# SYNCC-IN/hyperscanning-signal-analysis

Hardware: AMD Instinct MI355X
Metric: MVAR+ffDTF windows/sec, 2x32-ch dyad p=8, 256 freqs (higher is better)
Workload: dtype f64; 1 GPU; C2: 1 dyad(s)/GPU, 2x32 ch @500 Hz, 10 min, 2 s windows 50% overlap (599 windows per dyad), MVAR p=8, 256 freqs 0.5-128 Hz; dyads_per_gpu=1, k1=hop blocks summed once, shared by the overlapping windows (hop 500), k2=block Levinson-Whittle recursion, one workgroup per window, one launch, normalisation=inside K3 (rows of window w by workgroups of window w+lag), parallelism=dyad-sharded x1, gather=none

## Files before the change

hyperscanning_signal_analysis_amd/csrc/capi.hip:

```cpp
#include "../../include/hypermvar.h"
#include "hmv_kernels.h"

#include <atomic>
#include <cmath>
#include <cstdio>
#include <cstdlib>
#include <cstring>

namespace {
thread_local char g_err[256] = "";

int fail(int code, const char* msg) {
  snprintf(g_err, sizeof(g_err), "%s", msg);
  return code;
}
int pad_of(int m) { return (m < 1 || m > HMV_MAX_CHANNELS) ? -1 : ((m + 15) / 16) * 16; }
inline hipStream_t S(void* s) { return reinterpret_cast<hipStream_t>(s); }
inline size_t align256(size_t b) { return (b + 255) & ~size_t(255); }

constexpr int N_TUNE = 6;
struct TuneRange { long long lo, hi; };
constexpr TuneRange kTuneRange[N_TUNE] = {{0, 0}, {0, 1 << 20}, {0, 3}, {0, 2}, {0, 3}, {0, 140000}};
long long env_knob(const char* name, int key) {
  const char* e = getenv(name);
// ... 126 lines not shown
    const int64_t need = ens_q_tiles(n_items, n, p, grid_hop, grid_nwin) * (int64_t)(p + 1) * mp * mp;
    if (!workspace || workspace_doubles < need) return fail(-7, "hmv_lagcov_ensemble_f64: workspace too small");
  }
  hmv::LagcovEnsArgs a{};
  a.x = x; a.rec_stride = rec_stride; a.ld = ld; a.T = T;
  a.trial_rec = reinterpret_cast<const long long*>(trial_rec);
  a.trial_start = reinterpret_cast<const long long*>(trial_start);
  a.group_ptr = reinterpret_cast<const long long*>(group_ptr);
  a.item_group = reinterpret_cast<const long long*>(item_group);
  a.item_offset = reinterpret_cast<const long long*>(item_offset);
  a.n_items = n_items; a.m = m; a.n = n; a.p = p; a.R = R;
  if (shared) { a.it0 = 0; a.nwin = grid_nwin; a.hop = grid_hop; a.k = (int)(n / grid_hop); a.Q = workspace; }
  return hmv::launch_lagcov_ensemble(a, mp, shared, S(stream));
}

int hmv_yw_solve_f64(const double* R, int64_t n_items, int m, int p, double* ws, double* ar, double* V,
                     double* vq_logdet, int32_t* info, int64_t flags, void* stream) {
  const int mp = pad_of(m);
  if (mp < 0) return fail(-1, "hmv_yw_solve_f64: channel count must be in 1..64");
  if (p < 1 || p > HMV_MAX_ORDER) return fail(-2, "hmv_yw_solve_f64: model order must be in 1..32");
  if (!R || !ws || !ar || !V || !info || n_items < 0) return fail(-4, "hmv_yw_solve_f64: null pointer");
  hmv::YwArgs a{};
  a.R = R; a.n_items = n_items; a.m = m; a.p = p; a.ws = ws; a.ar = ar; a.V = V;
  a.Vq_logdet = vq_logdet; a.info = info; a.tiled = (flags & HMV_FLAG_YW_TILED) ? 1 : ((flags & HMV_FLAG_YW_ONE_LAUNCH) ? 0 : -1);
  return hmv::launch_yw(a, mp, S(stream));
}

namespace {
double crit_factor(int crit, int n) {
  return crit == 0 ? 2.0 : (crit == 1 ? 2.0 * log(log((double)n)) : log((double)n));
}
}

int hmv_yw_solve_auto_f64(const double* R, int64_t n_items, int m, int pmax, int n, int crit, double* ws, double* ar,
                          double* V, int32_t* order_out, double* crit_out, double* vq_logdet, int32_t* info, int64_t flags,
                          void* stream) {
  const int mp = pad_of(m);
  if (mp < 0) return fail(-1, "hmv_yw_solve_auto_f64: channel count must be in 1..64");
  if (pmax < 1 || pmax > HMV_MAX_ORDER) return fail(-2, "hmv_yw_solve_auto_f64: largest model order must be in 1..32");
  if (n <= pmax) return fail(-3, "hmv_yw_solve_auto_f64: window shorter than the largest model order");
// ... 197 lines not shown
  if (const int64_t t = hmv::tuning(HMV_TUNE_NORM_LAG)) lag = t;
  return lag < 8 ? 8 : lag;
}
}

int64_t hmv_tf_ffdtf_workspace_bytes(int64_t n_items, int m, int p, int F) {
  const int mp = pad_of(m);
  if (mp < 0 || n_items < 0 || p < 1 || F < 1) return -1;
  return (int64_t)tf_ff_layout(n_items, mp, p, F).total;
}

namespace {
int tf_ffdtf_impl(const char* who, const double* ar, int64_t n_items, int m, int p, const double* tw, int F, double* ffdtf,
                  double* band_out, const int32_t* bin_lo, const int32_t* bin_hi, int n_bands, double* den, double* H,
                  int32_t* info, double pivot_tau, void* workspace, int64_t workspace_bytes, int64_t flags,
                  void* ev_k3_start, void* ev_k3_stop, void* stream) {
  auto failw = [&](int code, const char* msg) {
    char buf[200];
    snprintf(buf, sizeof(buf), "%s: %s", who, msg);
    return fail(code, buf);
  };
  const int mp = pad_of(m);
  const bool bands = (band_out != nullptr);
  if (mp < 0) return failw(-1, "channel count must be in 1..64");
  if (p < 1) return failw(-2, "model order must be >= 1");
  if (n_items == 0) return 0;
  if (!ar || !tw || (!ffdtf && !bands) || !den || !info || !workspace || n_items < 0 || F < 1)
    return failw(-4, "null pointer / empty grid");
  if (!(pivot_tau > 0.0) || pivot_tau > 1.0) return failw(-6, "pivot_tau must be in (0, 1]");
  if (bands) {
    if (!bin_lo || !bin_hi || n_bands < 1) return failw(-4, "band bins missing");
    if (F % 32 != 0 || F > hmv::tf_band_max_F(mp) || (flags & HMV_FLAG_UNFUSED_NORM))
      return failw(-10, "in-kernel band sums need F % 32 == 0, F within the row worker's LDS block and the fused normalisation");
  }
  const TfFfWs w = tf_ff_layout(n_items, mp, p, F, bands);
  if ((int64_t)w.total > workspace_bytes) return failw(-7, "workspace too small");
  char* base = static_cast<char*>(workspace);
  const size_t t = (size_t)mp * mp;
  hmv::TfArgs a{};
  a.ar = ar; a.arx = reinterpret_cast<double*>(base + w.off_arx); a.tw = tw;
  a.P = reinterpret_cast<double*>(base + w.off_P); a.rowsum = reinterpret_cast<double*>(base + w.off_rowsum);
  a.H = H;
  a.info = info; a.n_items = n_items; a.F = F; a.p = p; a.m = m; a.tau = pivot_tau;
  const bool fused = bands || (!(flags & HMV_FLAG_UNFUSED_NORM) && (F % 16 == 0) && (reinterpret_cast<uintptr_t>(ffdtf) % 16 == 0));
  const int64_t lag = norm_lag_items(mp, F);
  const int64_t n_fused = fused ? n_items : 0;
  if (n_fused > 0) {
    a.ff = bands ? nullptr : ffdtf; a.den = den; a.fuse_items = n_fused; a.lag = (int)lag;
    if (bands) {
      a.bands = band_out; a.band_lo = reinterpret_cast<const int*>(bin_lo); a.band_hi = reinterpret_cast<const int*>(bin_hi);
      a.nb = n_bands;
    }
    a.wcount = reinterpret_cast<int*>(base + w.off_cnt);
    a.ready = a.wcount + n_items;
    a.missed = a.ready + n_items;
// ... 195 lines not shown
  double* Qb = reinterpret_cast<double*>(base + w.off_Q);
  double* ws = reinterpret_cast<double*>(base + w.off_ws);
  double* ar = reinterpret_cast<double*>(base + w.off_ar);
  double* V = reinterpret_cast<double*>(base + w.off_V);
  void* tfws = base + w.off_tf;
  double* den = reinterpret_cast<double*>(base + w.off_den);
  double* tw = reinterpret_cast<double*>(base + w.off_tw);
  const bool k3_bands = bands && a.measure == MEAS_FFDTF;
  const int64_t tfws_bytes = (int64_t)tf_ff_layout(a.chunk, mp, a.p, a.F, k3_bands).total;
  rc = hmv_twiddles_f64(a.freqs, a.F, a.fs, a.p, tw, st0);
  const size_t ws_item = (size_t)hmv_yw_workspace_doubles(a.m, a.p);
  for (int64_t ci = 0; ci < n_chunks && rc == 0; ++ci) {
    const int64_t i0 = ci * a.chunk;
    const int64_t c = (a.n_items - i0 < a.chunk) ? (a.n_items - i0) : a.chunk;
    double* ar_c = a.ar_out ? a.ar_out + (size_t)i0 * t * a.p : ar;
    double* V_c = a.V_out ? a.V_out + (size_t)i0 * t : V;
    if (a.ens) {
      hmv::LagcovEnsArgs ea{};
      ea.x = a.x; ea.rec_stride = a.rec_stride; ea.ld = a.ld; ea.T = a.ens->T;
      ea.trial_rec = reinterpret_cast<const long long*>(a.ens->trial_rec);
      ea.trial_start = reinterpret_cast<const long long*>(a.ens->trial_start);
      ea.group_ptr = reinterpret_cast<const long long*>(a.ens->group_ptr);
      ea.item_group = reinterpret_cast<const long long*>(a.item_rec + i0);
      ea.item_offset = reinterpret_cast<const long long*>(a.item_start + i0);
      ea.n_items = c; ea.m = a.m; ea.n = a.n; ea.p = a.p; ea.R = R;
      if (ens_shared) {
        ea.it0 = i0; ea.nwin = a.grid_nwin; ea.hop = a.grid_hop; ea.k = (int)(a.n / a.grid_hop); ea.Q = Qb;
      }
      rc = hmv::launch_lagcov_ensemble(ea, mp, ens_shared, st0);
    } else if (regular) {
// ... 25 lines not shown
    const int64_t c0 = (split && tiled && c >= 16) ? (c + 1) / 2 : c, c1 = c - c0;
    if (c1 > 0 && !automatic) {
      int hrc = (int)hipEventRecord(fj->fork, st0);
      if (!hrc) hrc = (int)hipStreamWaitEvent(st1, fj->fork, 0);
      if (hrc) { rc = hrc; break; }
      rc = hmv_yw_solve_f64(R + (size_t)c0 * (a.p + 1) * t, c1, a.m, a.p, ws + (size_t)c0 * ws_item,
                            ar_c + (size_t)c0 * t * a.p, V_c + (size_t)c0 * t, nullptr, a.info_yw + i0 + c0, yw_flags, st1);
      hrc = (int)hipEventRecord(fj->join, st1);
      if (!hrc) hrc = (int)hipStreamWaitEvent(st0, fj->join, 0);
      if (hrc) {
        (void)hipStreamSynchronize(st1);
        if (!rc) rc = hrc;
      }
      if (rc) break;
    }
    if (!automatic) rc = hmv_yw_solve_f64(R, c0, a.m, a.p, ws, ar_c, V_c, nullptr, a.info_yw + i0, yw_flags, st0);
    if (rc) break;
    const bool last = (ci == n_chunks - 1);
    double* Hc = a.S_out ? reinterpret_cast<double*>(base + w.off_H) : nullptr;
    double* full_c = (a.measure == MEAS_FFDTF) ? nullptr
                     : bands ? reinterpret_cast<double*>(base + w.off_full) : a.ffdtf + (size_t)i0 * a.m * a.m * a.F;
    if (a.measure == MEAS_GPDC) {
      rc = hmv::launch_gpdc_sliding(ar_c, V_c, tw, full_c, c, a.F, a.m, mp, a.p, st0);
    } else {
      rc = tf_ffdtf_impl(a.who, ar_c, c, a.m, a.p, tw, a.F,
                         k3_bands ? nullptr : (full_c ? full_c : a.ffdtf + (size_t)i0 * a.m * a.m * a.F),
                         k3_bands ? a.band_out + (size_t)i0 * a.m * a.m * a.n_bands : nullptr, a.bin_lo, a.bin_hi,
                         a.n_bands, den, Hc, a.info_tf + (size_t)i0 * a.F, a.pivot_tau, tfws, tfws_bytes, a.flags,
                         last ? a.ev_k3_start : nullptr, last ? a.ev_k3_stop : nullptr, st0);
    }
    if (!rc && a.measure == MEAS_DDTF) {
      hmv::DdtfArgs da{};
      da.ar = ar_c; da.V = V_c; da.info_yw = a.info_yw + i0;
      da.B = reinterpret_cast<double*>(base + w.off_B); da.G = reinterpret_cast<double*>(base + w.off_G);
      da.freqs = a.freqs; da.fs = a.fs; da.ff = full_c; da.out = full_c;
      da.n_items = c; da.F = a.F; da.m = a.m; da.p = a.p;
      rc = hmv::launch_ddtf_sliding(da, mp, st0);
    }
    if (!rc && a.measure != MEAS_FFDTF && bands)
      rc = hmv::launch_band_sums(full_c, reinterpret_cast<const int*>(a.bin_lo), reinterpret_cast<const int*>(a.bin_hi),
                                 a.band_out + (size_t)i0 * a.m * a.m * a.n_bands, c * (long long)a.m * a.m, a.F,
                                 a.n_bands, st0);
    if (!rc && a.S_out) {
      hmv::SpecArgs sa;
// ... 293 lines not shown
```

hyperscanning_signal_analysis_amd/csrc/hmv_kernels.h:

```cpp
#pragma once
#include <hip/hip_runtime.h>
#include <stdint.h>

namespace hmv {

long long tuning(int key);

struct LagcovArgs {
  const double* x;
  long long rec_stride;
  long long ld;
  const long long* item_rec;
  const long long* item_start;
  long long n_items;
  int m, n, p;
  double* R;
  int blocks;
  long long blk_first, blk_T;
};
int launch_lagcov(const LagcovArgs& a, int m_pad, hipStream_t st);
struct LagcombArgs {
  const double* Q;
  const double* x;
  long long ld, first, hop, T;
// ... 22 lines not shown
long long lagcov_ensemble_q_tiles(long long n_items, long long nwin, int k);
int launch_lagcov_ensemble(const LagcovEnsArgs& a, int m_pad, bool shared, hipStream_t st);

struct YwArgs {
  const double* R;
  long long n_items;
  int m, p;
  double* ws;
  double* ar;
  double* V;
  double* Vq_logdet;
  int* info;
  int tiled;
  int only_guarded;
  const int* order;
};
struct YwAutoArgs {
  int n;
  double crit_c;
  int* order_out;
  double* crit_out;
};
long long yw_ws_tiles(int p);
int launch_yw(const YwArgs& a, int m_pad, hipStream_t st);
int launch_yw_lwr(const YwArgs& a, int m_pad, hipStream_t st);
int launch_yw_lwr2(const YwArgs& a, int m_pad, hipStream_t st);
int launch_yw_auto(const YwArgs& a, const YwAutoArgs& s, int m_pad, hipStream_t st);
int launch_yw_guarded(const YwArgs& a, int m_pad, hipStream_t st);

struct TfArgs {
  const double* ar;
  const double* arx;
  const double* tw;
  const double* Zin;
  double* detph;
  double* P;
  double* rowsum;
  double* H;
  double* A;
  int* info;
  long long n_items;
  int F, p, m;
  double tau;
  double* ff;
  double* den;
  int* wcount;
  int* ready;
// ... 122 lines not shown
```

hyperscanning_signal_analysis_amd/csrc/tf_inv.hip:

```cpp
#include "hmv_common.h"
#include "hmv_kernels.h"

namespace hmv {

#ifndef HMV_K3_WGS
#define HMV_K3_WGS 4
#endif

#ifndef HMV_ROW_LOADS_SC1
#define HMV_ROW_LOADS_SC1 0
#endif

#define HMV_LDS_FENCE()                                     \
  do {                                                      \
    __builtin_amdgcn_fence(__ATOMIC_RELEASE, "wavefront");  \
    __builtin_amdgcn_wave_barrier();                        \
    __builtin_amdgcn_fence(__ATOMIC_ACQUIRE, "wavefront");  \
  } while (0)

#ifdef HMV_STAMP
#define HMV_T(idx)                                                                     \
  do {                                                                                 \
    __builtin_amdgcn_sched_barrier(0);                                                 \
    unsigned long long t_;                                                             \
// ... 192 lines not shown
        if (b < nbp && b0 + b < nb) {
          const double t0 = row16_sum_dpp(acc[b][0]), t1 = row16_sum_dpp(acc[b][1]);
          if (c == 0 && j0 < m) ow[b] = t0;
          if (c == 0 && j0 + 1 < m) ow[nb + b] = t1;
        }
      }
    }
  }
}

template <int NT>
__global__ void __launch_bounds__(64 * NT) norm_missed_kernel(TfArgs a) {
  __shared__ double lds[2 * TfLds<NT>::TOTAL];
  static_assert(NormLds<NT>::DOUBLES <= 2 * TfLds<NT>::TOTAL, "normaliser tiles do not fit");
  const int n = a.missed[0];
  const long long tail0 = a.fuse_items > a.lag ? a.fuse_items - a.lag : 0;
  const long long total = n + (a.fuse_items - tail0) * a.m;
  for (long long k = blockIdx.x; k < total; k += gridDim.x) {
    int item, i;
    if (k < n) {
      const int e = a.missed[1 + k];
      item = e / (16 * NT);
      i = e % (16 * NT);
    } else {
      const long long r = k - n;
      item = (int)(tail0 + r / a.m);
      i = (int)(r % a.m);
    }
    if (a.bands) band_row<NT>(a, item, i, lds, 2 * TfLds<NT>::TOTAL, (int)threadIdx.x);
    else normalise_row<NT>(a, item, i, lds, (int)threadIdx.x);
    __syncthreads();
  }
}

template <int NT, bool GEN, bool BANDS = true>
__device__ __forceinline__ void tf_outputs(const TfArgs& a, const int item, const int f, const long long gw, const int w,
                                           const int wv, double (&re)[NT][4], double (&im)[NT][4], double2* smem,
                                           double* rsum, const int* s_orig, int* s_flag, const double* s_det
#ifdef HMV_STAMP
                                           , unsigned long long (&tsum)[8], unsigned long long& tlast
#endif
) {
  constexpr int MP = 16 * NT, NG = NT;
  using L = TfLds<NT>;
  constexpr int NR = L::NRING;
  int& s_info = *s_flag;
  int lo;
  asm volatile("v_mbcnt_lo_u32_b32 %0, -1, 0\n\tv_mbcnt_hi_u32_b32 %0, -1, %0" : "=v"(lo));
  const int rowo = 4 * ((lo >> 2) & 3) + (lo >> 4), jo = lo & 3;
  const int tid = 64 * wv + lo;
  int oc[4];
#pragma unroll
  for (int Jl = 0; Jl < 4; ++Jl) oc[Jl] = s_orig[4 * (Jl * NT + w) + jo];
  if (w == 0 && lo == 0) {
    a.info[gw] = s_info;
    if constexpr (GEN) {
      if (a.detph) {
        a.detph[2 * gw] = s_det[0];
        a.detph[2 * gw + 1] = s_det[1];
      }
    }
  }

  if (a.H) {
    double2* Ho = reinterpret_cast<double2*>(a.H) + (size_t)gw * MP * MP + (size_t)rowo * MP;
#pragma unroll
    for (int Ig = 0; Ig < NG; ++Ig)
#pragma unroll
      for (int Jl = 0; Jl < 4; ++Jl) Ho[(size_t)(16 * Ig) * MP + oc[Jl]] = make_double2(re[Ig][Jl], im[Ig][Jl]);
  }
  if (a.P) {
    double* rs = rsum + w * MP + rowo;
    const bool publish = !GEN && (a.ff != nullptr || a.bands != nullptr) && item < a.fuse_items;
    if (!publish) {
      double* Po = a.P + (size_t)gw * MP * MP + (size_t)rowo * MP;
#pragma unroll
      for (int Ig = 0; Ig < NG; ++Ig) {
        double acc = 0.0;
#pragma unroll
        for (int Jl = 0; Jl < 4; ++Jl) {
          const double v = re[Ig][Jl] * re[Ig][Jl] + im[Ig][Jl] * im[Ig][Jl];
          Po[(size_t)(16 * Ig) * MP + oc[Jl]] = v;
          acc += v;
        }
        acc += dpp_f64<0xB1>(acc);
        acc += dpp_f64<0x4E>(acc);
// ... 59 lines not shown
            __builtin_amdgcn_fence(__ATOMIC_ACQUIRE, "agent");
            asm volatile("s_waitcnt vmcnt(0)" ::: "memory");
          }
          s_info = last;
        }
        __syncthreads();
        HMV_T(5);
        if (s_info != 0) {
          window_denominators<NT>(a, item, nlds, tid);
          asm volatile("s_waitcnt vmcnt(0)" ::: "memory");
          __syncthreads();
          if (tid == 0) __hip_atomic_store(a.ready + item, 1, __ATOMIC_RELAXED, __HIP_MEMORY_SCOPE_AGENT);
        }
      }
      const int wl = item - a.lag;
      if (wl >= 0 && wl < a.fuse_items - a.lag && f < a.m) {
        __syncthreads();
        if (tid == 0) {
          const int rdy = __hip_atomic_load(a.ready + wl, __ATOMIC_RELAXED, __HIP_MEMORY_SCOPE_AGENT);
          if (!rdy) {
            for (int i = f; i < a.m; i += a.F) {
              const int pos = __hip_atomic_fetch_add(a.missed, 1, __ATOMIC_RELAXED, __HIP_MEMORY_SCOPE_AGENT);
              a.missed[1 + pos] = wl * MP + i;
            }
          }
          s_info = rdy;
        }
        __syncthreads();
        HMV_T(6);
        if (s_info != 0) {
          if (BANDS && a.bands) {
            if constexpr (BANDS)
              for (int i = f; i < a.m; i += a.F) band_row<NT>(a, wl, i, nlds, 2 * L::TOTAL, tid);
          } else {
            for (int i = f; i < a.m; i += a.F) normalise_row<NT>(a, wl, i, nlds, tid);
          }
        }
      }
    }
  }
#ifdef HMV_STAMP
  HMV_T(7);
  if (a.stamps && lo == 0) {
    for (int k = 0; k < 8; ++k) a.stamps[(gw * NT + wv) * 8 + k] = tsum[k];
  }
#endif
}

template <int NT, bool GEN>
__global__ void __launch_bounds__(64 * NT, (NT == 4) ? HMV_K3_WGS : 2) tf_inv_kernel(TfArgs a) {
  constexpr int MP = 16 * NT, NG = NT, NSTEP = MP / 4;
  using L = TfLds<NT>;
  constexpr int NR = L::NRING;
  __shared__ double2 smem[L::TOTAL];
  __shared__ int s_orig[MP];
  __shared__ __attribute__((aligned(16))) int s_swp[NR][4];
  __shared__ int s_info;
  __shared__ double s_det[2];

  const int l = lane_id();
  const int wv = uni(threadIdx.x >> 6);
  const int w = (wv + (int)((blockIdx.x * 2654435761u) >> 20)) % NT;
  const int item = uni((int)(blockIdx.x / (unsigned)a.F));
  const int f = uni((int)(blockIdx.x - (unsigned)item * (unsigned)a.F));
  const long long gw = (long long)item * a.F + f;
  const int p = a.p;
  const int i = l >> 4, b = (l >> 2) & 3, j = l & 3;
  const int rowl = 4 * b + i;
  const int colw = 4 * w + j;

  double2* Pbuf = smem;
  double2* Nbuf = Pbuf + L::PBUF;
  double2* Srow = Nbuf + NR * L::NBUF;
  double2* swapb = Srow + L::SROW + wv * 32;
  double* rsum = reinterpret_cast<double*>(Srow + L::SROW + L::SWAPB);

  double re[NG][4], im[NG][4];
#ifdef HMV_STAMP
  unsigned long long tsum[8] = {0, 0, 0, 0, 0, 0, 0, 0}, tlast;
  asm volatile("s_memtime %0\n\ts_waitcnt lgkmcnt(0)" : "=s"(tlast)::"memory");
#endif

  if constexpr (GEN) {
    const double2* Zi = reinterpret_cast<const double2*>(a.Zin) + (size_t)gw * MP * MP + (size_t)rowl * MP + colw;
#pragma unroll
    for (int Ig = 0; Ig < NG; ++Ig)
#pragma unroll
      for (int Jl = 0; Jl < 4; ++Jl) {
        const double2 v = Zi[(size_t)(16 * Ig) * MP + 4 * NT * Jl];
        re[Ig][Jl] = v.x;
        im[Ig][Jl] = v.y;
      }
  } else {
    const int P2 = (p + 1) >> 1;
    const double2* ax = reinterpret_cast<const double2*>(a.arx) +
                        ((size_t)item * NT + w) * (size_t)(NG * 4 * 64) * P2 + l;
    const double* tw = a.tw + (size_t)f * p * 2;
#pragma unroll
    for (int Ig = 0; Ig < NG; ++Ig)
#pragma unroll
      for (int Jl = 0; Jl < 4; ++Jl) {
        re[Ig][Jl] = (16 * Ig + rowl == 4 * NT * Jl + colw) ? 1.0 : 0.0;
        im[Ig][Jl] = 0.0;
      }
    auto chunk = [&](auto hc_tag, int h0) __attribute__((always_inline)) {
      constexpr int HC = decltype(hc_tag)::value;
      constexpr int NB = NG * 4, DEPTH = (HC == 4) ? 3 : 8;
      double zr[2 * HC], zi[2 * HC];
// ... 241 lines not shown
        HMV_LDS_FENCE();
      }
    }
  };
  auto take_panel = [&](auto tc, auto jc) __attribute__((always_inline)) {
    constexpr int t = decltype(tc)::value, J = decltype(jc)::value;
    const double2* Nt = Nbuf + (t % NR) * L::NBUF;
#pragma unroll
    for (int Ig = 0; Ig < NG; ++Ig) {
      const double2 v = Nt[(16 * Ig + rowl) * 4 + j];
      re[Ig][J] = v.x;
      im[Ig][J] = v.y;
    }
  };

  if (w == 0) factor_panel(std::integral_constant<int, 0>{}, std::integral_constant<int, 0>{});
  HMV_T(1);
  __syncthreads();
  HMV_T(2);
  static_for<NSTEP>([&](auto sc) __attribute__((always_inline)) {
    constexpr int s = decltype(sc)::value;
    constexpr int own = s % NT, Js = s / NT;
    constexpr bool has_next = (s + 1 < NSTEP);
    constexpr int nxt = (s + 1) % NT, Jn = has_next ? (s + 1) / NT : 0;
    if (has_next && w == nxt) __builtin_amdgcn_s_setprio(3);
    if constexpr (s >= 1) {
      constexpr int t = s - 1;
      double ar_[NG], ai_[NG];
#pragma unroll
      for (int Ig = 0; Ig < NG; ++Ig) ar_[Ig] = ai_[Ig] = 0.0;
      if (w == own) load_n(std::integral_constant<int, t>{}, ar_, ai_);
      static_for<4>([&](auto jc) __attribute__((always_inline)) {
        constexpr int Jl = decltype(jc)::value;
        if constexpr (Jl != Js && !(NT == 1 && Jl == t / NT)) {
          if (w == own) update_block(std::integral_constant<int, t>{}, jc, ar_, ai_);
        }
      });
    }
    HMV_T(3);
    __builtin_amdgcn_sched_barrier(0);
    double nr[NG], ni[NG];
    load_n(sc, nr, ni);
    interchange(sc);
    HMV_T(3);
    const bool is_nxt = has_next && (w == nxt);
    if (w == own) take_panel(sc, std::integral_constant<int, Js>{});
    if (is_nxt || !(w == own && Jn == Js)) update_block(sc, std::integral_constant<int, Jn>{}, nr, ni);
    static_for<4>([&](auto jc) __attribute__((always_inline)) {
      constexpr int Jl = decltype(jc)::value;
      if constexpr (Jl != Jn) {
        if (!is_nxt && !(w == own && Jl == Js)) update_block(sc, jc, nr, ni);
      }
    });
    HMV_T(3);
    __builtin_amdgcn_sched_barrier(0);
    if (is_nxt) factor_panel(std::integral_constant<int, s + 1>{}, std::integral_constant<int, Jn>{});
    HMV_T(1);
    __syncthreads();
    HMV_T(2);
  });

  HMV_T(3);
  tf_outputs<NT, GEN, (NT < 4)>(a, item, f, gw, w, wv, re, im, smem, rsum, s_orig, &s_info, s_det
#ifdef HMV_STAMP
                      , tsum, tlast
#endif
  );
}

#ifndef HMV_K3A_INC
#define HMV_K3A_INC "tf_inv64_body.inc"
#endif
#include HMV_K3A_INC
#ifndef HMV_K3A_WGS
#ifdef HMV_STAMP
// ... 15 lines not shown
  const int item = uni((int)(blockIdx.x / (unsigned)a.F));
  const int f = uni((int)(blockIdx.x - (unsigned)item * (unsigned)a.F));
  const long long gw = (long long)item * a.F + f;
  if (w == 0) {
    const int l = lane_id();
    s_orig[l] = l;
    if (l == 0) *s_flag = 0;
  }
  const int p = a.p, P2 = (p + 1) >> 1;
  const double* arx = a.arx + ((size_t)item * NT + w) * (size_t)(16 * 64 * 2) * P2;
  const double* tw = a.tw + (size_t)f * p * 2;
  const double tau = a.tau;
  const unsigned ldsbase = (unsigned)(uintptr_t)lds;
  double acc[32];
#ifdef HMV_STAMP
  unsigned long long tsum[8] = {0, 0, 0, 0, 0, 0, 0, 0}, tlast = 0, q0, q1, q2, q3;
  unsigned tl32;
  K3A_BODY_STAMPED(acc, arx, tw, p, w, tau, ldsbase, q0, q1, q2, q3, tl32);
  {
    const unsigned long long d[8] = {q0 & 0xffffffffull, q0 >> 32, q1 & 0xffffffffull, q1 >> 32,
                                     q2 & 0xffffffffull, q2 >> 32, q3 & 0xffffffffull, q3 >> 32};
    tsum[0] = d[0]; tsum[2] = d[1]; tsum[3] = d[2] + d[3] + d[4]; tsum[1] = d[5] + d[6] + d[7];
    unsigned long long now;
    asm volatile("s_memtime %0\n\ts_waitcnt lgkmcnt(0)" : "=s"(now)::"memory");
    tlast = (now & ~0xffffffffull) | tl32;
    if (tlast > now) tlast -= 0x100000000ull;
    if (a.stamps && lane_id() == 0) {
      unsigned long long* det = a.stamps + ((size_t)a.n_items * a.F * NT + (size_t)(gw * NT + wv)) * 8;
      for (int k = 0; k < 8; ++k) det[k] = d[k];
    }
  }
#else
  K3A_BODY(acc, arx, tw, p, w, tau, ldsbase);
#endif
  double re[NT][4], im[NT][4];
#pragma unroll
  for (int Ig = 0; Ig < 4; ++Ig)
#pragma unroll
    for (int Jl = 0; Jl < 4; ++Jl) {
      re[Ig][Jl] = acc[2 * (4 * Ig + Jl)];
      im[Ig][Jl] = acc[2 * (4 * Ig + Jl) + 1];
    }
  double2* smem = reinterpret_cast<double2*>(lds);
  double* rsum = reinterpret_cast<double*>(lds + K3A_RSUM);
  tf_outputs<NT, false>(a, item, f, gw, w, wv, re, im, smem, rsum, s_orig, s_flag, nullptr
#ifdef HMV_STAMP
                        , tsum, tlast
#endif
// ... 48 lines not shown
    case 64: return (2 * TfLds<4>::TOTAL) & ~31;
  }
  return 0;
}

long long tf_workspace_doubles(long long n_items, int m_pad, int p) {
  return n_items * (long long)m_pad * m_pad * 2 * ((p + 1) / 2);
}

int launch_tf_inv(const TfArgs& a_in, int m_pad, hipStream_t st, hipEvent_t ev_start, hipEvent_t ev_stop) {
  TfArgs a = a_in;
  if (a.n_items == 0 || a.F == 0) return 0;
  const bool fused = ((a.ff != nullptr || a.bands != nullptr) && a.fuse_items > 0);
  if (fused) {
    if (!a.P || !a.den || !a.wcount || !a.ready || !a.missed || a.lag < 1) return -3;
    if (a.bands && (!a.band_lo || !a.band_hi || a.nb < 1 || a.F % 32 != 0 || a.F > tf_band_max_F(m_pad) || a.A)) return -3;
    if (const hipError_t e = hipMemsetAsync(a.wcount, 0, sizeof(int) * (2 * (size_t)a.n_items + 1), st)) return (int)e;
  } else {
    a.ff = nullptr;
    a.bands = nullptr;
  }
  const long long n = a.n_items * (long long)a.F;
  const dim3 grid((unsigned)n);
  const long long slots = a.n_items * (long long)m_pad * m_pad * ((a.p + 1) / 2);
  const dim3 pgrid((unsigned)((slots + 255) / 256));
  double* arx = const_cast<double*>(a.arx);
  switch (m_pad) {
    case 16: hipLaunchKernelGGL(ar_pack_kernel<1>, pgrid, dim3(256), 0, st, a.ar, arx, a.n_items, a.p); break;
    case 32: hipLaunchKernelGGL(ar_pack_kernel<2>, pgrid, dim3(256), 0, st, a.ar, arx, a.n_items, a.p); break;
    case 48: hipLaunchKernelGGL(ar_pack_kernel<3>, pgrid, dim3(256), 0, st, a.ar, arx, a.n_items, a.p); break;
    case 64: hipLaunchKernelGGL(ar_pack_kernel<4>, pgrid, dim3(256), 0, st, a.ar, arx, a.n_items, a.p); break;
    default: return -1;
  }
  if (ev_start)
    if (const hipError_t e = hipEventRecord(ev_start, st)) return (int)e;
  switch (m_pad) {
    case 16: hipLaunchKernelGGL((tf_inv_kernel<1, false>), grid, dim3(64), 0, st, a); break;
    case 32: hipLaunchKernelGGL((tf_inv_kernel<2, false>), grid, dim3(128), 0, st, a); break;
    case 48: hipLaunchKernelGGL((tf_inv_kernel<3, false>), grid, dim3(192), 0, st, a); break;
    case 64:
      if (tuning(5) > 0) {
        (void)hipFuncSetAttribute(reinterpret_cast<const void*>(&tf_inv64_asm_kernel), hipFuncAttributeMaxDynamicSharedMemorySize,
                                  (int)tuning(5));
        (void)hipFuncSetAttribute(reinterpret_cast<const void*>(&tf_inv_kernel<4, false>),
                                  hipFuncAttributeMaxDynamicSharedMemorySize, (int)tuning(5));
      }
      if ((tuning(3 ) != 1 || a.bands != nullptr) && a.A == nullptr)
        hipLaunchKernelGGL(tf_inv64_asm_kernel, grid, dim3(256), (unsigned)tuning(5 ), st, a);
      else
        hipLaunchKernelGGL((tf_inv_kernel<4, false>), grid, dim3(256), (unsigned)tuning(5), st, a);
      break;
  }
  if (ev_stop)
    if (const hipError_t e = hipEventRecord(ev_stop, st)) return (int)e;
  if (fused) {
    const long long tail_rows = (a.fuse_items > a.lag ? a.lag : a.fuse_items) * a.m;
    const dim3 mgrid((unsigned)(tail_rows > 2048 ? 2048 : (tail_rows < 256 ? 256 : tail_rows)));
    switch (m_pad) {
      case 16: hipLaunchKernelGGL(norm_missed_kernel<1>, mgrid, dim3(64), 0, st, a); break;
      case 32: hipLaunchKernelGGL(norm_missed_kernel<2>, mgrid, dim3(128), 0, st, a); break;
      case 48: hipLaunchKernelGGL(norm_missed_kernel<3>, mgrid, dim3(192), 0, st, a); break;
      case 64: hipLaunchKernelGGL(norm_missed_kernel<4>, mgrid, dim3(256), 0, st, a); break;
    }
  }
  return (int)hipGetLastError();
}

int launch_cinv(const TfArgs& a_in, int m_pad, hipStream_t st) {
  TfArgs a = a_in;
  a.ff = nullptr;
  a.bands = nullptr;
// ... 16 lines not shown
```

hyperscanning_signal_analysis_amd/csrc/yw_auto.hip:

```cpp
#include "yw_lwr_core.h"

namespace hmv {

template <int NT>
__global__ void __launch_bounds__(256, 3) yw_auto_kernel(YwArgs a, YwAutoArgs sel) {
  yw_lwr_body<NT, true, true>(a, sel);
}

int launch_yw_auto(const YwArgs& a_in, const YwAutoArgs& sel, int m_pad, hipStream_t st) {
  YwArgs a = a_in;
  if (a.n_items == 0) return 0;
  a.order = nullptr;
  a.only_guarded = 0;
  const dim3 grid((unsigned)a.n_items), block(256);
  switch (m_pad) {
    case 16: hipLaunchKernelGGL((yw_auto_kernel<1>), grid, block, 0, st, a, sel); break;
    case 32: hipLaunchKernelGGL((yw_auto_kernel<2>), grid, block, 0, st, a, sel); break;
    case 48: hipLaunchKernelGGL((yw_auto_kernel<3>), grid, block, 0, st, a, sel); break;
    case 64: hipLaunchKernelGGL((yw_auto_kernel<4>), grid, block, 0, st, a, sel); break;
    default: return -1;
  }
  if (const int rc = (int)hipGetLastError()) return rc;
  a.order = sel.order_out;
  return launch_yw_guarded(a, m_pad, st);
}

}
```

hyperscanning_signal_analysis_amd/csrc/yw_lwr_core.h:

```cpp
#pragma once
#include "yw_common.h"

namespace hmv {

#ifndef HMV_LWR_GUARD
#define HMV_LWR_GUARD 1e-7
#endif

template <int NT, bool VQ, bool AUTO>
__device__ __forceinline__ void yw_lwr_body(const YwArgs& a, const YwAutoArgs& sel) {
  static_assert(VQ || !AUTO, "the selecting form needs every log det Vf_q");
  constexpr int MP = 16 * NT, KH = MP / 2, SH = KH + 6, NIW = NT, NJ = NT, TILE = MP * MP;
  constexpr int NV = (MP * KH / 2 + 255) / 256;
  constexpr int SI = YwCfg<NT>::S;
  constexpr int GEMM_D = 2 * MP * SH, INV_D = MP * SI, BUF_D = GEMM_D > INV_D ? GEMM_D : INV_D;
  __shared__ __attribute__((aligned(16))) double buf[BUF_D];
  __shared__ double Pb[2 * MP * 4];
  __shared__ double Nb[4 * MP * 4];
  __shared__ int s_info;
  __shared__ double s_ld[4];
  __shared__ double s_pm[4 + 4 * 4];
  __shared__ int s_guard;
  __shared__ double s_logdet, s_best;
  __shared__ int s_qstar, s_take;
// ... 218 lines not shown
  };
  auto emit = [&](const double* Aq, int q) __attribute__((always_inline)) {
    double* ar = a.ar + (size_t)item * TILE * p;
    const int total = TILE * q, de = 256 / q, dk = 256 - de * q;
    int e = (int)threadIdx.x / q, k = (int)threadIdx.x - e * q;
    for (int idx = threadIdx.x; idx < total; idx += 256) {
      ar[(size_t)e * p + k] = Aq[(size_t)k * TILE + e];
      e += de;
      k += dk;
      if (k >= q) {
        k -= q;
        ++e;
      }
    }
  };
  auto select = [&](int q) __attribute__((always_inline)) {
    if (threadIdx.x == 0) {
      const double ld = s_logdet;
      const double crit = ld + ((sel.crit_c * (double)q) * (double)(a.m * a.m)) / (double)sel.n;
      if (sel.crit_out) sel.crit_out[(size_t)item * p + (q - 1)] = crit;
      if (a.Vq_logdet) a.Vq_logdet[(size_t)item * p + (q - 1)] = ld;
      const int take = (crit < s_best) ? 1 : 0;
      if (take) {
        s_best = crit;
        s_qstar = q;
      }
      s_take = take;
    }
    __syncthreads();
    if (s_take) {
// ... 97 lines not shown
      k += dk;
      k = (k >= p) ? k - p : k;
    }
    if (qs == 0) {
      double* Vo = a.V + (size_t)item * TILE;
      for (int idx = threadIdx.x; idx < TILE; idx += 256) Vo[idx] = R[idx];
    }
    return;
  }
  load_tile(g, Vf, false);
  store_tile(a.V + (size_t)item * TILE, g);
  if (threadIdx.x == 0) {
    a.info[item] = s_info;
    *yw_guard_ptr(a.ws, item, p, TILE) = (s_info == 0) ? s_guard : 0;
  }
  emit(Agen[p & 1], p);
}

}
```

hyperscanning_signal_analysis_amd/csrc/yw_solve.hip:

```cpp
#include "yw_common.h"
#include <cstdlib>

namespace hmv {

long long yw_ws_tiles(int p) { return yw_ws_tiles_d(p); }

struct YwPtrs {
  const double* R;
  double *Yt, *Lt, *Dinv, *Zt;
};
template <int MP>
__device__ __forceinline__ YwPtrs yw_ptrs(const YwArgs& a, long long item, int p) {
  constexpr int TILE = MP * MP;
  double* ws = a.ws + (size_t)item * yw_ws_tiles_d(a.p) * TILE;
  const long long ntri = yw_tri(p + 1, 0);
  YwPtrs q;
  q.R = a.R + (size_t)item * (a.p + 1) * TILE;
  q.Yt = ws;
  q.Lt = ws + ntri * TILE;
  q.Dinv = ws + 2 * ntri * TILE;
  q.Zt = q.Dinv + (size_t)p * TILE;
  return q;
}

// ... 262 lines not shown
#pragma unroll
      for (int ii = 0; ii < NIW; ++ii)
#pragma unroll
        for (int J = 0; J < NJ; ++J) g[ii][J] -= acc[ii][J];
    }
    store_tile(q.Zt + (size_t)b * TILE, g);
    __syncthreads();
  }
  const int pa = a.p;
  double* ar = a.ar + (size_t)item * TILE * pa;
  const int total = TILE * pa;
  for (int idx = threadIdx.x; idx < total; idx += 256) {
    const int e = idx / pa, k = idx - e * pa;
    ar[idx] = (k < p) ? q.Zt[(size_t)k * TILE + e] : 0.0;
  }
}

template <int NT>
static int launch_yw_nt(const YwArgs& a, hipStream_t st) {
  const int p = a.p;
  const unsigned n = (unsigned)a.n_items;
  if (const hipError_t e = hipMemsetAsync(a.info, 0, sizeof(int) * a.n_items, st)) return (int)e;
  for (int tb = 0; tb <= p; ++tb) {
    const dim3 grid(((n + 7) / 8) * 8 * (unsigned)(p - tb + 1));
    if (a.Vq_logdet && tb == p) hipLaunchKernelGGL((yw_window_kernel<NT, true, 2>), grid, dim3(256), 0, st, a, tb);
    else hipLaunchKernelGGL((yw_window_kernel<NT, false, 2>), grid, dim3(256), 0, st, a, tb);
  }
  hipLaunchKernelGGL((yw_window_kernel<NT, false, 1>), dim3(n), dim3(256), 0, st, a, 0);
  return (int)hipGetLastError();
}
// ... 3 lines not shown
  a.only_guarded = 1;
  a.tiled = 0;
  a.Vq_logdet = nullptr;
  if (a.n_items == 0) return 0;
  const dim3 grid((unsigned)a.n_items), block(256);
  switch (m_pad) {
    case 16: hipLaunchKernelGGL((yw_window_kernel<1, false>), grid, block, 0, st, a, 0); break;
    case 32: hipLaunchKernelGGL((yw_window_kernel<2, false>), grid, block, 0, st, a, 0); break;
    case 48: hipLaunchKernelGGL((yw_window_kernel<3, false>), grid, block, 0, st, a, 0); break;
    case 64: hipLaunchKernelGGL((yw_window_kernel<4, false>), grid, block, 0, st, a, 0); break;
    default: return -1;
  }
  return (int)hipGetLastError();
}

int launch_yw(const YwArgs& a_in, int m_pad, hipStream_t st) {
  YwArgs a = a_in;
  a.only_guarded = 0;
  a.order = nullptr;
  if (a.n_items == 0) return 0;
  const long long form = tuning(4 );
  if (a.tiled < 0 && form != 1) {
    int rc = launch_yw_lwr(a, m_pad, st);
    if (rc) return rc;
    a.only_guarded = 1;
    a.tiled = 0;
  }
  const bool one_launch = a.tiled == 0 || (a.tiled < 0 && !(m_pad == 64 && a.n_items >= 128));
  if (one_launch) {
    if (!a.only_guarded)
      if (const hipError_t e = hipMemsetAsync(a.info, 0, sizeof(int) * a.n_items, st)) return (int)e;
    const dim3 grid((unsigned)a.n_items), block(256);
    const bool vq = (a.Vq_logdet != nullptr);
    switch (m_pad) {
      case 16: if (vq) hipLaunchKernelGGL((yw_window_kernel<1, true>), grid, block, 0, st, a, 0);
               else hipLaunchKernelGGL((yw_window_kernel<1, false>), grid, block, 0, st, a, 0); break;
      case 32: if (vq) hipLaunchKernelGGL((yw_window_kernel<2, true>), grid, block, 0, st, a, 0);
               else hipLaunchKernelGGL((yw_window_kernel<2, false>), grid, block, 0, st, a, 0); break;
      case 48: if (vq) hipLaunchKernelGGL((yw_window_kernel<3, true>), grid, block, 0, st, a, 0);
// ... 19 lines not shown
```

Before: 61370 windows/s.

## Emit packed AR coefficients from K2 and fold normaliser tail into K3 grid

The Levinson-Whittle solver now writes the AR coefficients directly in the packed layout that the transfer-function kernel consumes. This removes the separate ar_pack kernel launch and, when nothing else needs the plain AR array, its global write and re-read. The trailing normalisation rows that the missed-row kernel used to handle are now done by extra K3 workgroups appended to the grid, which skip the inversion and only run the normaliser. In exchange the code gains more branching, a scratch AR buffer for the guarded fallback path, and a new requirement that fuse_items equals n_items.

```diff
diff --git a/hyperscanning_signal_analysis_amd/csrc/capi.hip b/hyperscanning_signal_analysis_amd/csrc/capi.hip
--- a/hyperscanning_signal_analysis_amd/csrc/capi.hip
+++ b/hyperscanning_signal_analysis_amd/csrc/capi.hip
@@ -164,16 +164,26 @@
   return hmv::launch_lagcov_ensemble(a, mp, shared, S(stream));
 }
 
+namespace {
+int yw_tiled_of(int64_t flags) { return (flags & HMV_FLAG_YW_TILED) ? 1 : ((flags & HMV_FLAG_YW_ONE_LAUNCH) ? 0 : -1); }
+int yw_solve_impl(const double* R, int64_t n_items, int m, int p, double* ws, double* ar, double* arx, double* ar_scratch,
+                  double* V, double* vq_logdet, int32_t* info, int64_t flags, void* stream) {
+  const int mp = pad_of(m);
+  if (mp < 0) return fail(-1, "hmv_yw_solve_f64: channel count must be in 1..64");
+  if (p < 1 || p > HMV_MAX_ORDER) return fail(-2, "hmv_yw_solve_f64: model order must be in 1..32");
+  if (!R || !ws || (!ar && !(arx && ar_scratch)) || !V || !info || n_items < 0) return fail(-4, "hmv_yw_solve_f64: null pointer");
+  hmv::YwArgs a{};
+  a.R = R; a.n_items = n_items; a.m = m; a.p = p; a.ws = ws; a.ar = ar; a.V = V;
+  a.arx = arx; a.ar_scratch = ar_scratch;
+  a.Vq_logdet = vq_logdet; a.info = info; a.tiled = yw_tiled_of(flags);
+  return hmv::launch_yw(a, mp, S(stream));
+}
+}
+
 int hmv_yw_solve_f64(const double* R, int64_t n_items, int m, int p, double* ws, double* ar, double* V,
                      double* vq_logdet, int32_t* info, int64_t flags, void* stream) {
-  const int mp = pad_of(m);
-  if (mp < 0) return fail(-1, "hmv_yw_solve_f64: channel count must be in 1..64");
-  if (p < 1 || p > HMV_MAX_ORDER) return fail(-2, "hmv_yw_solve_f64: model order must be in 1..32");
-  if (!R || !ws || !ar || !V || !info || n_items < 0) return fail(-4, "hmv_yw_solve_f64: null pointer");
-  hmv::YwArgs a{};
-  a.R = R; a.n_items = n_items; a.m = m; a.p = p; a.ws = ws; a.ar = ar; a.V = V;
-  a.Vq_logdet = vq_logdet; a.info = info; a.tiled = (flags & HMV_FLAG_YW_TILED) ? 1 : ((flags & HMV_FLAG_YW_ONE_LAUNCH) ? 0 : -1);
-  return hmv::launch_yw(a, mp, S(stream));
+  if (!ar) return fail(-4, "hmv_yw_solve_f64: null pointer");
+  return yw_solve_impl(R, n_items, m, p, ws, ar, nullptr, nullptr, V, vq_logdet, info, flags, stream);
 }
 
 namespace {
@@ -401,7 +411,7 @@
 int tf_ffdtf_impl(const char* who, const double* ar, int64_t n_items, int m, int p, const double* tw, int F, double* ffdtf,
                   double* band_out, const int32_t* bin_lo, const int32_t* bin_hi, int n_bands, double* den, double* H,
                   int32_t* info, double pivot_tau, void* workspace, int64_t workspace_bytes, int64_t flags,
-                  void* ev_k3_start, void* ev_k3_stop, void* stream) {
+                  void* ev_k3_start, void* ev_k3_stop, void* stream, bool arx_ready = false) {
   auto failw = [&](int code, const char* msg) {
     char buf[200];
     snprintf(buf, sizeof(buf), "%s: %s", who, msg);
@@ -412,7 +422,7 @@
   if (mp < 0) return failw(-1, "channel count must be in 1..64");
   if (p < 1) return failw(-2, "model order must be >= 1");
   if (n_items == 0) return 0;
-  if (!ar || !tw || (!ffdtf && !bands) || !den || !info || !workspace || n_items < 0 || F < 1)
+  if ((!ar && !arx_ready) || !tw || (!ffdtf && !bands) || !den || !info || !workspace || n_items < 0 || F < 1)
     return failw(-4, "null pointer / empty grid");
   if (!(pivot_tau > 0.0) || pivot_tau > 1.0) return failw(-6, "pivot_tau must be in (0, 1]");
   if (bands) {
@@ -425,7 +435,7 @@
   char* base = static_cast<char*>(workspace);
   const size_t t = (size_t)mp * mp;
   hmv::TfArgs a{};
-  a.ar = ar; a.arx = reinterpret_cast<double*>(base + w.off_arx); a.tw = tw;
+  a.ar = ar; a.arx = reinterpret_cast<double*>(base + w.off_arx); a.arx_ready = arx_ready ? 1 : 0; a.tw = tw;
   a.P = reinterpret_cast<double*>(base + w.off_P); a.rowsum = reinterpret_cast<double*>(base + w.off_rowsum);
   a.H = H;
   a.info = info; a.n_items = n_items; a.F = F; a.p = p; a.m = m; a.tau = pivot_tau;
@@ -651,6 +661,10 @@
     const int64_t i0 = ci * a.chunk;
     const int64_t c = (a.n_items - i0 < a.chunk) ? (a.n_items - i0) : a.chunk;
     double* ar_c = a.ar_out ? a.ar_out + (size_t)i0 * t * a.p : ar;
+    const bool k2_packs = !automatic && a.measure != MEAS_GPDC && hmv::yw_writes_arx(yw_tiled_of(a.flags));
+    double* arx_c = k2_packs ? reinterpret_cast<double*>(static_cast<char*>(tfws) + tf_ff_layout(c, mp, a.p, a.F, k3_bands).off_arx)
+                             : nullptr;
+    const bool ar_read = a.ar_out || a.measure != MEAS_FFDTF;
     double* V_c = a.V_out ? a.V_out + (size_t)i0 * t : V;
     if (a.ens) {
       hmv::LagcovEnsArgs ea{};
@@ -706,7 +720,9 @@
       }
       if (rc) break;
     }
-    if (!automatic) rc = hmv_yw_solve_f64(R, c0, a.m, a.p, ws, ar_c, V_c, nullptr, a.info_yw + i0, yw_flags, st0);
+    if (!automatic)
+      rc = yw_solve_impl(R, c0, a.m, a.p, ws, (k2_packs && !ar_read) ? nullptr : ar_c, arx_c, k2_packs ? ar : nullptr, V_c,
+                         nullptr, a.info_yw + i0, yw_flags, st0);
     if (rc) break;
     const bool last = (ci == n_chunks - 1);
     double* Hc = a.S_out ? reinterpret_cast<double*>(base + w.off_H) : nullptr;
@@ -719,7 +735,7 @@
                          k3_bands ? nullptr : (full_c ? full_c : a.ffdtf + (size_t)i0 * a.m * a.m * a.F),
                          k3_bands ? a.band_out + (size_t)i0 * a.m * a.m * a.n_bands : nullptr, a.bin_lo, a.bin_hi,
                          a.n_bands, den, Hc, a.info_tf + (size_t)i0 * a.F, a.pivot_tau, tfws, tfws_bytes, a.flags,
-                         last ? a.ev_k3_start : nullptr, last ? a.ev_k3_stop : nullptr, st0);
+                         last ? a.ev_k3_start : nullptr, last ? a.ev_k3_stop : nullptr, st0, k2_packs);
     }
     if (!rc && a.measure == MEAS_DDTF) {
       hmv::DdtfArgs da{};
diff --git a/hyperscanning_signal_analysis_amd/csrc/hmv_kernels.h b/hyperscanning_signal_analysis_amd/csrc/hmv_kernels.h
--- a/hyperscanning_signal_analysis_amd/csrc/hmv_kernels.h
+++ b/hyperscanning_signal_analysis_amd/csrc/hmv_kernels.h
@@ -60,7 +60,10 @@
   int tiled;
   int only_guarded;
   const int* order;
-};
+  double* arx;
+  double* ar_scratch;
+};
+bool yw_writes_arx(int tiled);
 struct YwAutoArgs {
   int n;
   double crit_c;
@@ -77,6 +80,7 @@
 struct TfArgs {
   const double* ar;
   const double* arx;
+  int arx_ready;
   const double* tw;
   const double* Zin;
   double* detph;
diff --git a/hyperscanning_signal_analysis_amd/csrc/tf_inv.hip b/hyperscanning_signal_analysis_amd/csrc/tf_inv.hip
--- a/hyperscanning_signal_analysis_amd/csrc/tf_inv.hip
+++ b/hyperscanning_signal_analysis_amd/csrc/tf_inv.hip
@@ -230,19 +230,9 @@
   __shared__ double lds[2 * TfLds<NT>::TOTAL];
   static_assert(NormLds<NT>::DOUBLES <= 2 * TfLds<NT>::TOTAL, "normaliser tiles do not fit");
   const int n = a.missed[0];
-  const long long tail0 = a.fuse_items > a.lag ? a.fuse_items - a.lag : 0;
-  const long long total = n + (a.fuse_items - tail0) * a.m;
-  for (long long k = blockIdx.x; k < total; k += gridDim.x) {
-    int item, i;
-    if (k < n) {
-      const int e = a.missed[1 + k];
-      item = e / (16 * NT);
-      i = e % (16 * NT);
-    } else {
-      const long long r = k - n;
-      item = (int)(tail0 + r / a.m);
-      i = (int)(r % a.m);
-    }
+  for (int k = blockIdx.x; k < n; k += gridDim.x) {
+    const int e = a.missed[1 + k];
+    const int item = e / (16 * NT), i = e % (16 * NT);
     if (a.bands) band_row<NT>(a, item, i, lds, 2 * TfLds<NT>::TOTAL, (int)threadIdx.x);
     else normalise_row<NT>(a, item, i, lds, (int)threadIdx.x);
     __syncthreads();
@@ -261,6 +251,7 @@
   using L = TfLds<NT>;
   constexpr int NR = L::NRING;
   int& s_info = *s_flag;
+  const bool tail = !GEN && item >= a.n_items;
   int lo;
   asm volatile("v_mbcnt_lo_u32_b32 %0, -1, 0\n\tv_mbcnt_hi_u32_b32 %0, -1, %0" : "=v"(lo));
   const int rowo = 4 * ((lo >> 2) & 3) + (lo >> 4), jo = lo & 3;
@@ -268,7 +259,7 @@
   int oc[4];
 #pragma unroll
   for (int Jl = 0; Jl < 4; ++Jl) oc[Jl] = s_orig[4 * (Jl * NT + w) + jo];
-  if (w == 0 && lo == 0) {
+  if (!tail && w == 0 && lo == 0) {
     a.info[gw] = s_info;
     if constexpr (GEN) {
       if (a.detph) {
@@ -278,14 +269,14 @@
     }
   }
 
-  if (a.H) {
+  if (a.H && !tail) {
     double2* Ho = reinterpret_cast<double2*>(a.H) + (size_t)gw * MP * MP + (size_t)rowo * MP;
 #pragma unroll
     for (int Ig = 0; Ig < NG; ++Ig)
 #pragma unroll
       for (int Jl = 0; Jl < 4; ++Jl) Ho[(size_t)(16 * Ig) * MP + oc[Jl]] = make_double2(re[Ig][Jl], im[Ig][Jl]);
   }
-  if (a.P) {
+  if (a.P && !tail) {
     double* rs = rsum + w * MP + rowo;
     const bool publish = !GEN && (a.ff != nullptr || a.bands != nullptr) && item < a.fuse_items;
     if (!publish) {
@@ -375,7 +366,7 @@
         }
       }
       const int wl = item - a.lag;
-      if (wl >= 0 && wl < a.fuse_items - a.lag && f < a.m) {
+      if (wl >= 0 && wl < a.fuse_items - (tail ? 0 : a.lag) && f < a.m) {
         __syncthreads();
         if (tid == 0) {
           const int rdy = __hip_atomic_load(a.ready + wl, __ATOMIC_RELAXED, __HIP_MEMORY_SCOPE_AGENT);
@@ -402,7 +393,7 @@
   }
 #ifdef HMV_STAMP
   HMV_T(7);
-  if (a.stamps && lo == 0) {
+  if (a.stamps && lo == 0 && !tail) {
     for (int k = 0; k < 8; ++k) a.stamps[(gw * NT + wv) * 8 + k] = tsum[k];
   }
 #endif
@@ -426,6 +417,7 @@
   const int f = uni((int)(blockIdx.x - (unsigned)item * (unsigned)a.F));
   const long long gw = (long long)item * a.F + f;
   const int p = a.p;
+  const bool inverting = GEN || item < a.n_items;
   const int i = l >> 4, b = (l >> 2) & 3, j = l & 3;
   const int rowl = 4 * b + i;
   const int colw = 4 * w + j;
@@ -452,7 +444,7 @@
         re[Ig][Jl] = v.x;
         im[Ig][Jl] = v.y;
       }
-  } else {
+  } else if (inverting) {
     const int P2 = (p + 1) >> 1;
     const double2* ax = reinterpret_cast<const double2*>(a.arx) +
                         ((size_t)item * NT + w) * (size_t)(NG * 4 * 64) * P2 + l;
@@ -724,51 +716,53 @@
     }
   };
 
-  if (w == 0) factor_panel(std::integral_constant<int, 0>{}, std::integral_constant<int, 0>{});
-  HMV_T(1);
-  __syncthreads();
-  HMV_T(2);
-  static_for<NSTEP>([&](auto sc) __attribute__((always_inline)) {
-    constexpr int s = decltype(sc)::value;
-    constexpr int own = s % NT, Js = s / NT;
-    constexpr bool has_next = (s + 1 < NSTEP);
-    constexpr int nxt = (s + 1) % NT, Jn = has_next ? (s + 1) / NT : 0;
-    if (has_next && w == nxt) __builtin_amdgcn_s_setprio(3);
-    if constexpr (s >= 1) {
-      constexpr int t = s - 1;
-      double ar_[NG], ai_[NG];
-#pragma unroll
-      for (int Ig = 0; Ig < NG; ++Ig) ar_[Ig] = ai_[Ig] = 0.0;
-      if (w == own) load_n(std::integral_constant<int, t>{}, ar_, ai_);
-      static_for<4>([&](auto jc) __attribute__((always_inline)) {
-        constexpr int Jl = decltype(jc)::value;
-        if constexpr (Jl != Js && !(NT == 1 && Jl == t / NT)) {
-          if (w == own) update_block(std::integral_constant<int, t>{}, jc, ar_, ai_);
-        }
-      });
-    }
-    HMV_T(3);
-    __builtin_amdgcn_sched_barrier(0);
-    double nr[NG], ni[NG];
-    load_n(sc, nr, ni);
-    interchange(sc);
-    HMV_T(3);
-    const bool is_nxt = has_next && (w == nxt);
-    if (w == own) take_panel(sc, std::integral_constant<int, Js>{});
-    if (is_nxt || !(w == own && Jn == Js)) update_block(sc, std::integral_constant<int, Jn>{}, nr, ni);
-    static_for<4>([&](auto jc) __attribute__((always_inline)) {
-      constexpr int Jl = decltype(jc)::value;
-      if constexpr (Jl != Jn) {
-        if (!is_nxt && !(w == own && Jl == Js)) update_block(sc, jc, nr, ni);
-      }
-    });
-    HMV_T(3);
-    __builtin_amdgcn_sched_barrier(0);
-    if (is_nxt) factor_panel(std::integral_constant<int, s + 1>{}, std::integral_constant<int, Jn>{});
+  if (inverting) {
+    if (w == 0) factor_panel(std::integral_constant<int, 0>{}, std::integral_constant<int, 0>{});
     HMV_T(1);
     __syncthreads();
     HMV_T(2);
-  });
+    static_for<NSTEP>([&](auto sc) __attribute__((always_inline)) {
+      constexpr int s = decltype(sc)::value;
+      constexpr int own = s % NT, Js = s / NT;
+      constexpr bool has_next = (s + 1 < NSTEP);
+      constexpr int nxt = (s + 1) % NT, Jn = has_next ? (s + 1) / NT : 0;
+      if (has_next && w == nxt) __builtin_amdgcn_s_setprio(3);
+      if constexpr (s >= 1) {
+        constexpr int t = s - 1;
+        double ar_[NG], ai_[NG];
+#pragma unroll
+        for (int Ig = 0; Ig < NG; ++Ig) ar_[Ig] = ai_[Ig] = 0.0;
+        if (w == own) load_n(std::integral_constant<int, t>{}, ar_, ai_);
+        static_for<4>([&](auto jc) __attribute__((always_inline)) {
+          constexpr int Jl = decltype(jc)::value;
+          if constexpr (Jl != Js && !(NT == 1 && Jl == t / NT)) {
+            if (w == own) update_block(std::integral_constant<int, t>{}, jc, ar_, ai_);
+          }
+        });
+      }
+      HMV_T(3);
+      __builtin_amdgcn_sched_barrier(0);
+      double nr[NG], ni[NG];
+      load_n(sc, nr, ni);
+      interchange(sc);
+      HMV_T(3);
+      const bool is_nxt = has_next && (w == nxt);
+      if (w == own) take_panel(sc, std::integral_constant<int, Js>{});
+      if (is_nxt || !(w == own && Jn == Js)) update_block(sc, std::integral_constant<int, Jn>{}, nr, ni);
+      static_for<4>([&](auto jc) __attribute__((always_inline)) {
+        constexpr int Jl = decltype(jc)::value;
+        if constexpr (Jl != Jn) {
+          if (!is_nxt && !(w == own && Jl == Js)) update_block(sc, jc, nr, ni);
+        }
+      });
+      HMV_T(3);
+      __builtin_amdgcn_sched_barrier(0);
+      if (is_nxt) factor_panel(std::integral_constant<int, s + 1>{}, std::integral_constant<int, Jn>{});
+      HMV_T(1);
+      __syncthreads();
+      HMV_T(2);
+    });
+  }
 
   HMV_T(3);
   tf_outputs<NT, GEN, (NT < 4)>(a, item, f, gw, w, wv, re, im, smem, rsum, s_orig, &s_info, s_det
@@ -814,10 +808,15 @@
   const unsigned ldsbase = (unsigned)(uintptr_t)lds;
   double acc[32];
 #ifdef HMV_STAMP
-  unsigned long long tsum[8] = {0, 0, 0, 0, 0, 0, 0, 0}, tlast = 0, q0, q1, q2, q3;
-  unsigned tl32;
-  K3A_BODY_STAMPED(acc, arx, tw, p, w, tau, ldsbase, q0, q1, q2, q3, tl32);
-  {
+  unsigned long long tsum[8] = {0, 0, 0, 0, 0, 0, 0, 0}, tlast = 0, q0 = 0, q1 = 0, q2 = 0, q3 = 0;
+  unsigned tl32 = 0;
+  if (item < a.n_items) {
+    K3A_BODY_STAMPED(acc, arx, tw, p, w, tau, ldsbase, q0, q1, q2, q3, tl32);
+  } else {
+#pragma unroll
+    for (int k = 0; k < 32; ++k) acc[k] = 0.0;
+  }
+  if (item < a.n_items) {
     const unsigned long long d[8] = {q0 & 0xffffffffull, q0 >> 32, q1 & 0xffffffffull, q1 >> 32,
                                      q2 & 0xffffffffull, q2 >> 32, q3 & 0xffffffffull, q3 >> 32};
     tsum[0] = d[0]; tsum[2] = d[1]; tsum[3] = d[2] + d[3] + d[4]; tsum[1] = d[5] + d[6] + d[7];
@@ -831,7 +830,12 @@
     }
   }
 #else
-  K3A_BODY(acc, arx, tw, p, w, tau, ldsbase);
+  if (item < a.n_items) {
+    K3A_BODY(acc, arx, tw, p, w, tau, ldsbase);
+  } else {
+#pragma unroll
+    for (int k = 0; k < 32; ++k) acc[k] = 0.0;
+  }
 #endif
   double re[NT][4], im[NT][4];
 #pragma unroll
@@ -910,23 +914,28 @@
   const bool fused = ((a.ff != nullptr || a.bands != nullptr) && a.fuse_items > 0);
   if (fused) {
     if (!a.P || !a.den || !a.wcount || !a.ready || !a.missed || a.lag < 1) return -3;
+    if (a.fuse_items != a.n_items) return -3;
     if (a.bands && (!a.band_lo || !a.band_hi || a.nb < 1 || a.F % 32 != 0 || a.F > tf_band_max_F(m_pad) || a.A)) return -3;
     if (const hipError_t e = hipMemsetAsync(a.wcount, 0, sizeof(int) * (2 * (size_t)a.n_items + 1), st)) return (int)e;
   } else {
     a.ff = nullptr;
     a.bands = nullptr;
   }
-  const long long n = a.n_items * (long long)a.F;
-  const dim3 grid((unsigned)n);
-  const long long slots = a.n_items * (long long)m_pad * m_pad * ((a.p + 1) / 2);
-  const dim3 pgrid((unsigned)((slots + 255) / 256));
-  double* arx = const_cast<double*>(a.arx);
-  switch (m_pad) {
-    case 16: hipLaunchKernelGGL(ar_pack_kernel<1>, pgrid, dim3(256), 0, st, a.ar, arx, a.n_items, a.p); break;
-    case 32: hipLaunchKernelGGL(ar_pack_kernel<2>, pgrid, dim3(256), 0, st, a.ar, arx, a.n_items, a.p); break;
-    case 48: hipLaunchKernelGGL(ar_pack_kernel<3>, pgrid, dim3(256), 0, st, a.ar, arx, a.n_items, a.p); break;
-    case 64: hipLaunchKernelGGL(ar_pack_kernel<4>, pgrid, dim3(256), 0, st, a.ar, arx, a.n_items, a.p); break;
-    default: return -1;
+  const long long tail_rows = fused ? (a.fuse_items > a.lag ? a.lag : a.fuse_items) * a.m : 0;
+  const long long n = a.n_items * (long long)a.F, n_trail = fused ? a.lag * (long long)a.F : 0;
+  if (n + n_trail > 0x7fffffffll) return -1;
+  const dim3 grid((unsigned)(n + n_trail));
+  if (m_pad != 16 && m_pad != 32 && m_pad != 48 && m_pad != 64) return -1;
+  if (!a.arx_ready) {
+    const long long slots = a.n_items * (long long)m_pad * m_pad * ((a.p + 1) / 2);
+    const dim3 pgrid((unsigned)((slots + 255) / 256));
+    double* arx = const_cast<double*>(a.arx);
+    switch (m_pad) {
+      case 16: hipLaunchKernelGGL(ar_pack_kernel<1>, pgrid, dim3(256), 0, st, a.ar, arx, a.n_items, a.p); break;
+      case 32: hipLaunchKernelGGL(ar_pack_kernel<2>, pgrid, dim3(256), 0, st, a.ar, arx, a.n_items, a.p); break;
+      case 48: hipLaunchKernelGGL(ar_pack_kernel<3>, pgrid, dim3(256), 0, st, a.ar, arx, a.n_items, a.p); break;
+      case 64: hipLaunchKernelGGL(ar_pack_kernel<4>, pgrid, dim3(256), 0, st, a.ar, arx, a.n_items, a.p); break;
+    }
   }
   if (ev_start)
     if (const hipError_t e = hipEventRecord(ev_start, st)) return (int)e;
@@ -950,7 +959,6 @@
   if (ev_stop)
     if (const hipError_t e = hipEventRecord(ev_stop, st)) return (int)e;
   if (fused) {
-    const long long tail_rows = (a.fuse_items > a.lag ? a.lag : a.fuse_items) * a.m;
     const dim3 mgrid((unsigned)(tail_rows > 2048 ? 2048 : (tail_rows < 256 ? 256 : tail_rows)));
     switch (m_pad) {
       case 16: hipLaunchKernelGGL(norm_missed_kernel<1>, mgrid, dim3(64), 0, st, a); break;
diff --git a/hyperscanning_signal_analysis_amd/csrc/yw_auto.hip b/hyperscanning_signal_analysis_amd/csrc/yw_auto.hip
--- a/hyperscanning_signal_analysis_amd/csrc/yw_auto.hip
+++ b/hyperscanning_signal_analysis_amd/csrc/yw_auto.hip
@@ -12,6 +12,7 @@
   if (a.n_items == 0) return 0;
   a.order = nullptr;
   a.only_guarded = 0;
+  a.arx = nullptr;
   const dim3 grid((unsigned)a.n_items), block(256);
   switch (m_pad) {
     case 16: hipLaunchKernelGGL((yw_auto_kernel<1>), grid, block, 0, st, a, sel); break;
diff --git a/hyperscanning_signal_analysis_amd/csrc/yw_lwr_core.h b/hyperscanning_signal_analysis_amd/csrc/yw_lwr_core.h
--- a/hyperscanning_signal_analysis_amd/csrc/yw_lwr_core.h
+++ b/hyperscanning_signal_analysis_amd/csrc/yw_lwr_core.h
@@ -256,6 +256,20 @@
       }
     }
   };
+  auto emit_packed = [&](const double* Aq) __attribute__((always_inline)) {
+    const int P2 = (p + 1) >> 1, nblk = NT * NT * 4 * P2;
+    const unsigned l = lane();
+    const unsigned e = (4 * ((l >> 2) & 3) + (l >> 4)) * MP + (l & 3);
+    f64x2* dst = reinterpret_cast<f64x2*>(a.arx) + (size_t)item * TILE * P2 + l;
+    for (int blk = wv; blk < nblk; blk += 4) {
+      const int h = blk % P2, r = blk / P2, Jl = r & 3, Ig = (r >> 2) % NT, w = (r >> 2) / NT;
+      const double* src = Aq + (size_t)(2 * h) * TILE + (16 * Ig * MP + 4 * (Jl * NT + w)) + e;
+      f64x2 v;
+      v.x = src[0];
+      v.y = (2 * h + 1 < p) ? src[TILE] : 0.0;
+      dst[(size_t)blk * 64] = v;
+    }
+  };
   auto select = [&](int q) __attribute__((always_inline)) {
     if (threadIdx.x == 0) {
       const double ld = s_logdet;
@@ -383,7 +397,9 @@
     a.info[item] = s_info;
     *yw_guard_ptr(a.ws, item, p, TILE) = (s_info == 0) ? s_guard : 0;
   }
-  emit(Agen[p & 1], p);
+  if constexpr (!AUTO)
+    if (a.arx) emit_packed(Agen[p & 1]);
+  if (AUTO || a.ar) emit(Agen[p & 1], p);
 }
 
 }
diff --git a/hyperscanning_signal_analysis_amd/csrc/yw_solve.hip b/hyperscanning_signal_analysis_amd/csrc/yw_solve.hip
--- a/hyperscanning_signal_analysis_amd/csrc/yw_solve.hip
+++ b/hyperscanning_signal_analysis_amd/csrc/yw_solve.hip
@@ -300,6 +300,26 @@
     const int e = idx / pa, k = idx - e * pa;
     ar[idx] = (k < p) ? q.Zt[(size_t)k * TILE + e] : 0.0;
   }
+  if constexpr (MODE == 0) {
+    if (a.only_guarded && a.arx) {
+      __syncthreads();
+      const int P2 = (pa + 1) >> 1, slots = TILE * P2;
+      f64x2* ax = reinterpret_cast<f64x2*>(a.arx) + (size_t)item * slots;
+      for (int idx = threadIdx.x; idx < slots; idx += 256) {
+        const int ln = idx & 63;
+        int r = idx >> 6;
+        const int h = r % P2; r /= P2;
+        const int Jl = r & 3; r >>= 2;
+        const int Ig = r % NT, w = r / NT;
+        const int row = 16 * Ig + 4 * ((ln >> 2) & 3) + (ln >> 4), col = 4 * (Jl * NT + w) + (ln & 3);
+        const double* e = ar + ((size_t)row * MP + col) * pa;
+        f64x2 v;
+        v.x = e[2 * h];
+        v.y = (2 * h + 1 < pa) ? e[2 * h + 1] : 0.0;
+        ax[idx] = v;
+      }
+    }
+  }
 }
 
 template <int NT>
@@ -333,15 +353,23 @@
   return (int)hipGetLastError();
 }
 
+bool yw_writes_arx(int tiled) {
+  const long long form = tuning(4 );
+  return tiled < 0 && form != 1 && form != 3;
+}
+
 int launch_yw(const YwArgs& a_in, int m_pad, hipStream_t st) {
   YwArgs a = a_in;
   a.only_guarded = 0;
   a.order = nullptr;
   if (a.n_items == 0) return 0;
+  if (a.arx && !yw_writes_arx(a.tiled)) return -1;
+  if (!a.ar && !(a.arx && a.ar_scratch)) return -1;
   const long long form = tuning(4 );
   if (a.tiled < 0 && form != 1) {
     int rc = launch_yw_lwr(a, m_pad, st);
     if (rc) return rc;
+    if (!a.ar) a.ar = a.ar_scratch;
     a.only_guarded = 1;
     a.tiled = 0;
   }
```

After: 61540 windows/s (median of 5 runs). About the same (+0.3%).
